# ZephirFXEC/HNanoSolver

Measured on AMD Instinct MI355X. Metric: solver substeps/sec (advect + 50 red-black SOR iterations + project) at N active voxels, higher is better.
Workload: dtype f32

## Files before the change

### hnanosolver_amd/csrc/hns_advect.hip

```cpp
#include <cstdlib>
#include <cstring>

#include "hns_device.hpp"

namespace hns {

struct Taps {
	int t[8];
	float fx, fy, fz;
};

constexpr unsigned kOutside = 0xFFFFE000u;
constexpr uint64_t kNarrowBytes = 0xFFFF0000ull;

__device__ __forceinline__ f3 ldv(const v4i& r, unsigned o4) {
	const v3f v = hns_buffer_load_v3f32(r, (int)(o4 + (o4 << 1)), 0, 0);
	return f3{v.x, v.y, v.z};
}
__device__ __forceinline__ float lds1(const v4i& r, unsigned o4) { return hns_buffer_load_f32(r, (int)o4, 0, 0); }

__device__ __forceinline__ void ld_zpair(const v4i& r, unsigned lo, unsigned hi, float& a, float& b) {
	const v2f32 v = hns_buffer_load_v2f32(r, (int)lo, 0, 0);
	a = v.x;
	b = v.y;
	if (hi != lo + 4u) b = lds1(r, hi);
}

struct GenericTabs {
	int nbr[27], base[27];
	__device__ __forceinline__ void set(int t, int nb) { nbr[t] = nb, base[t] = nb < 0 ? -1 : nb * 512; }
};
constexpr int kPadTab = 48;
struct NarrowTabs {
	int nbr[27];
	unsigned b4[27], b4p[kPadTab];
	__device__ __forceinline__ void set(int t, int nb) {
		const int ax = t / 9, ay = (t - 9 * ax) / 3, az = t - 9 * ax - 3 * ay;
		nbr[t] = nb, b4[t] = b4p[(ax * 4 + ay) * 4 + az] = nb < 0 ? kOutside : (unsigned)nb * 2048u;
	}
};

__device__ __forceinline__ int3 voxel_ijk(const int4 org, int n) { return int3{org.x + (n >> 6), org.y + ((n >> 3) & 7), org.z + (n & 7)}; }

template <class Tabs>
struct LeafVoxel {
	Tabs& tabs;
	const int n, leaf, idx;
	int4 org;
	int3 c;
	float px, py, pz;
	__device__ __forceinline__ LeafVoxel(const GridDev& g, Tabs& t) : tabs(t), n(threadIdx.x), leaf(launch_leaf(g, blockIdx.x)), idx(leaf * 512 + n) {}
	__device__ __forceinline__ void stage(const GridDev& g) {
		org = g.origins[leaf];
		if (threadIdx.x < 27) tabs.set(threadIdx.x, g.nbr27[leaf * 27 + threadIdx.x]);
		__syncthreads();
		c = voxel_ijk(org, n);
		px = (float)c.x, py = (float)c.y, pz = (float)c.z;
	}
};
typedef LeafVoxel<GenericTabs> GenericCtx;
typedef LeafVoxel<NarrowTabs> NarrowCtx;

__device__ __forceinline__ constexpr int tap_of(int q) { return ((q & 1) << 2) | (q & 2) | (q >> 2); }
template <int XS = 100, int YS = 10>
__device__ __forceinline__ constexpr int box_corner(int q) { return (q & 1) * XS + ((q >> 1) & 1) * YS + (q >> 2); }
__device__ __forceinline__ void tri_weights(float tx, float ty, float tz, float (&w)[8]) {
	const float itx = 1.0f - tx, ity = 1.0f - ty, itz = 1.0f - tz;
	const float w00 = itx * ity, w10 = tx * ity, w01 = itx * ty, w11 = tx * ty;
	w[0] = w00 * itz, w[1] = w10 * itz, w[2] = w01 * itz, w[3] = w11 * itz, w[4] = w00 * tz, w[5] = w10 * tz, w[6] = w01 * tz, w[7] = w11 * tz;
}
template <class T, class Lerp>
__device__ __forceinline__ T tri_nest_yx(const T (&z)[4], float fx, float fy, Lerp lerp) {
	const T y0 = lerp(z[0], z[1], fy), y1 = lerp(z[2], z[3], fy);
	return lerp(y0, y1, fx);
}
template <class T, class Lerp>
__device__ __forceinline__ T tri_nest(const T (&c)[8], float fx, float fy, float fz, Lerp lerp) {
	const T z[4] = {lerp(c[0], c[1], fz), lerp(c[2], c[3], fz), lerp(c[4], c[5], fz), lerp(c[6], c[7], fz)};
	return tri_nest_yx(z, fx, fy, lerp);
}
template <class T>
__device__ __forceinline__ T bfecc_limit(T phiOrig, const T (&nbr)[6], T phiForward, T phiCorr) {
	T mn = phiOrig, mx = phiOrig;
#pragma unroll
	for (int d = 0; d < 6; ++d) {
		mn = __builtin_elementwise_min(mn, nbr[d]);
		mx = __builtin_elementwise_max(mx, nbr[d]);
	}
	mn = __builtin_elementwise_min(mn, phiForward);
	mx = __builtin_elementwise_max(mx, phiForward);
	return __builtin_elementwise_max(mn, __builtin_elementwise_min(phiCorr, mx));
}
template <class Fetch>
__device__ __forceinline__ f3 bfecc_limit_v(const f3& vo, const f3& vf, const f3& vb, Fetch nbr) {
	float nx[6], ny[6], nz[6];
#pragma unroll
	for (int d = 0; d < 6; ++d) {
		const f3 t = nbr(d);
		nx[d] = t.x, ny[d] = t.y, nz[d] = t.z;
	}
	return f3{bfecc_limit(vo.x, nx, vf.x, vf.x + 0.5f * (vo.x - vb.x)), bfecc_limit(vo.y, ny, vf.y, vf.y + 0.5f * (vo.y - vb.y)),
	          bfecc_limit(vo.z, nz, vf.z, vf.z + 0.5f * (vo.z - vb.z))};
}

struct TapsB {
	unsigned o[8];
	float fx, fy, fz;
};

__device__ __forceinline__ Taps make_taps(const GridDev& g, const GenericCtx& C, float x, float y, float z) {
	Taps T;
	const int4 org = C.org;
	const int i = __float2int_rd(x), j = __float2int_rd(y), k = __float2int_rd(z);
	T.fx = x - (float)i;
	T.fy = y - (float)j;
	T.fz = z - (float)k;
	const int ax0 = (i >> 3) - (org.x >> 3) + 1, ax1 = ((i + 1) >> 3) - (org.x >> 3) + 1;
	const int ay0 = (j >> 3) - (org.y >> 3) + 1, ay1 = ((j + 1) >> 3) - (org.y >> 3) + 1;
	const int az0 = (k >> 3) - (org.z >> 3) + 1, az1 = ((k + 1) >> 3) - (org.z >> 3) + 1;
	const bool near = ((unsigned)ax0 <= 2u) & ((unsigned)ax1 <= 2u) & ((unsigned)ay0 <= 2u) & ((unsigned)ay1 <= 2u) & ((unsigned)az0 <= 2u) &
	                  ((unsigned)az1 <= 2u);
	if (near) {
		const int sx[2] = {ax0 * 9, ax1 * 9}, sy[2] = {ay0 * 3, ay1 * 3}, sz[2] = {az0, az1};
		const int lx[2] = {(i & 7) << 6, ((i + 1) & 7) << 6}, ly[2] = {(j & 7) << 3, ((j + 1) & 7) << 3}, lz[2] = {k & 7, (k + 1) & 7};
#pragma unroll
		for (int c = 0; c < 8; ++c) {
			const int di = c >> 2, dj = (c >> 1) & 1, dk = c & 1;
			const int b = C.tabs.base[sx[di] + sy[dj] + sz[dk]];
			T.t[c] = b < 0 ? -1 : b + (lx[di] | ly[dj] | lz[dk]);
		}
	} else {
		int any = 0;
		far_cell_taps(g, C.tabs.nbr, org, i, j, k, T.t);
#pragma unroll
		for (int c = 0; c < 8; ++c) any |= T.t[c];
		if (any < 0 && g.far_flag) *g.far_flag = 1;
	}
	return T;
}

__device__ __forceinline__ TapsB make_taps_b(const GridDev& g, const NarrowCtx& C, float x, float y, float z) {
	TapsB T;
	const int4 org = C.org;
	const int i = __float2int_rd(x), j = __float2int_rd(y), k = __float2int_rd(z);
	T.fx = x - (float)i;
	T.fy = y - (float)j;
	T.fz = z - (float)k;
	const unsigned dx = (unsigned)(i - (org.x - 8)), dy = (unsigned)(j - (org.y - 8)), dz = (unsigned)(k - (org.z - 8));
	if (max(dx, max(dy, dz)) < 23u) {
		const unsigned ex = dx + 1u, ey = dy + 1u, ez = dz + 1u;
		const unsigned X[2] = {(dx & 24u) << 3, (ex & 24u) << 3}, Y[2] = {(dy & 24u) << 1, (ey & 24u) << 1}, Z[2] = {(dz & 24u) >> 1, (ez & 24u) >> 1};
		const unsigned lx[2] = {(dx & 7u) << 8, (ex & 7u) << 8}, ly[2] = {(dy & 7u) << 5, (ey & 7u) << 5}, lz[2] = {(dz & 7u) << 2, (ez & 7u) << 2};
		const unsigned XY[4] = {X[0] | Y[0], X[0] | Y[1], X[1] | Y[0], X[1] | Y[1]};
		const unsigned lxy[4] = {lx[0] | ly[0], lx[0] | ly[1], lx[1] | ly[0], lx[1] | ly[1]};
// ... 174 lines not shown
	const v4i ru = field_rsrc(u, (unsigned)g.n_leaves * 6144u);
	const f3 vo = ldv(ru, (unsigned)C.idx << 2);
	C.stage(g);
	int cell;
	const unsigned off = box_shell_off<kVX, kVY>(tabs.b4, C.n, cell);
	velocity_box_store<kVP>(s_box, C.n, cell, velocity_box_load<kVX, kVY, kVP>(s_box, ru, C.n, vo, off));
	float sx = C.px - scaled_dt * vo.x, sy = C.py - scaled_dt * vo.y, sz = C.pz - scaled_dt * vo.z;
	f3 vf = {0.0f, 0.0f, 0.0f}, vb = {0.0f, 0.0f, 0.0f};
	__syncthreads();
#pragma unroll 1
	for (int pass = 0; pass < 2; ++pass) {
		const f3 v = sample_velocity(g, C, ru, s_box, sx, sy, sz);
		if (pass == 0) {
			vf = v;
			sx = sx + scaled_dt * v.x, sy = sy + scaled_dt * v.y, sz = sz + scaled_dt * v.z;
		} else {
			vb = v;
		}
	}
	const int ob = box_own<kVX, kVY>(C.n);
	st3(out, C.idx, bfecc_limit_v(vo, vf, vb, [&](int d) { return box_f3(s_box, ob + box_nbr<kVX, kVY>(d)); }));
}

template <bool COLL>
__global__ __launch_bounds__(512) void k_advect_vector(const GridDev g, const float* __restrict__ u, float* __restrict__ out,
                                                       const float* __restrict__ sdf, const float scaled_dt, const float inv_dx) {
	__shared__ GenericTabs tabs;
	GenericCtx C(g, tabs);
	C.stage(g);
	const int idx = C.idx;

	const f3 vo = ld3(u, idx);
	float sx = C.px - scaled_dt * vo.x, sy = C.py - scaled_dt * vo.y, sz = C.pz - scaled_dt * vo.z;
	float rx = C.px, ry = C.py, rz = C.pz;
	f3 vf = {0.0f, 0.0f, 0.0f}, vb = {0.0f, 0.0f, 0.0f};
#pragma unroll 1
	for (int pass = 0; pass < 2; ++pass) {
		Taps T = make_taps(g, C, sx, sy, sz);
		if (COLL) {
			if (tri_f_t(sdf, T) < 0.0f) {
				sx = rx, sy = ry, sz = rz;
				T = make_taps(g, C, sx, sy, sz);
			}
		}
		const f3 v = tri_v_t(u, T);
		if (pass == 0) {
			vf = v;
			rx = sx, ry = sy, rz = sz;
			sx = sx + scaled_dt * v.x, sy = sy + scaled_dt * v.y, sz = sz + scaled_dt * v.z;
		} else {
			vb = v;
		}
	}
	int nb[6];
	nbr6(tabs.base, C.leaf, C.n, nb);
	f3 vc = bfecc_limit_v(vo, vf, vb, [&](int d) { return ld3z(u, nb[d]); });

	if (COLL) {
		const float sv = sdf[idx];
		if (sv < 0.0f) {
			vc.x = vc.y = vc.z = 0.0f;
		} else if (sv < 0.1f) {
			const f3 nrm = sdf_normal(g, tabs.nbr, C.org, sdf, C.c.x, C.c.y, C.c.z, inv_dx);
			vc = no_slip_blend(vc, nrm, 1.0f - (sv / 1.5f));
		}
	}
	st3(out, idx, vc);
}


__global__ __launch_bounds__(512) void k_advect_scalar_n(const GridDev g, const float* __restrict__ u, const float* __restrict__ in, float* __restrict__ out,
                                                         const float scaled_dt) {
	__shared__ NarrowTabs tabs;
	NarrowCtx C(g, tabs);
	C.stage(g);
	const int n = C.n;
	const unsigned bytes1 = (unsigned)g.n_leaves * 2048u, own = (unsigned)C.idx << 2;
	const v4i ru = field_rsrc(u, bytes1 * 3u), rf = field_rsrc(in, bytes1);

	__shared__ float s_tile[kTile];
	const float phiOrig = lds1(rf, own);
	s_tile[n] = phiOrig;
	if (n < 384) s_tile[512 + n] = lds1(rf, halo_off(tabs.b4, n));
	const f3 vc = ldv(ru, own);
	float sx = C.px - scaled_dt * vc.x, sy = C.py - scaled_dt * vc.y, sz = C.pz - scaled_dt * vc.z;
	float phiForward = 0.0f, phiBackward = 0.0f;
#pragma unroll 1
	for (int pass = 0; pass < 2; ++pass) {
		const TapsB T = make_taps_b(g, C, sx, sy, sz);
		const float phi = tri_f_b(rf, T);
		if (pass == 0) {
			phiForward = phi;
			const f3 vf = tri_v_b(ru, T);
			sx = sx + scaled_dt * vf.x, sy = sy + scaled_dt * vf.y, sz = sz + scaled_dt * vf.z;
		} else {
			phiBackward = phi;
		}
	}
	const float error = phiOrig - phiBackward;
	__syncthreads();
	const float nv[6] = {s_tile[tile_nbr<0, -1>(n)], s_tile[tile_nbr<0, 1>(n)], s_tile[tile_nbr<1, -1>(n)], s_tile[tile_nbr<1, 1>(n)], s_tile[tile_nbr<2, -1>(n)], s_tile[tile_nbr<2, 1>(n)]};
	out[C.idx] = bfecc_limit(phiOrig, nv, phiForward, phiForward + 0.5f * error);
}

template <bool COLL>
__global__ __launch_bounds__(512) void k_advect_scalar(const GridDev g, const float* __restrict__ u, const float* __restrict__ in,
                                                       float* __restrict__ out, const float* __restrict__ sdf, const float scaled_dt) {
	__shared__ GenericTabs tabs;
	GenericCtx C(g, tabs);
	C.stage(g);
	const int idx = C.idx;

	const float phiOrig = in[idx];
	const f3 vc = ld3(u, idx);
	float sx = C.px - scaled_dt * vc.x, sy = C.py - scaled_dt * vc.y, sz = C.pz - scaled_dt * vc.z;
	float rx = C.px, ry = C.py, rz = C.pz;
	float phiForward = 0.0f, phiBackward = 0.0f;
#pragma unroll 1
	for (int pass = 0; pass < 2; ++pass) {
		Taps T = make_taps(g, C, sx, sy, sz);
		if (COLL) {
			if (tri_f_t(sdf, T) < 0.0f) {
				sx = rx, sy = ry, sz = rz;
				T = make_taps(g, C, sx, sy, sz);
			}
		}
		const float phi = tri_f_t(in, T);
		if (pass == 0) {
			phiForward = phi;
			const f3 vf = tri_v_t(u, T);
			rx = sx, ry = sy, rz = sz;
			sx = sx + scaled_dt * vf.x, sy = sy + scaled_dt * vf.y, sz = sz + scaled_dt * vf.z;
		} else {
			phiBackward = phi;
		}
	}
	const float error = phiOrig - phiBackward;
	int nb[6];
	nbr6(tabs.base, C.leaf, C.n, nb);
	float nv[6];
#pragma unroll
	for (int d = 0; d < 6; ++d) nv[d] = ldz(in, nb[d]);
	out[idx] = bfecc_limit(phiOrig, nv, phiForward, phiForward + 0.5f * error);
}


#define HNS_MAX_SCALARS 8
struct ScalarPtrs {
	const float* in[HNS_MAX_SCALARS];
	float* out[HNS_MAX_SCALARS];
	int n;
	const float* q4;
	float* q4_out[4];
};

__device__ __forceinline__ void interp_from_taps(const Taps& T, int oob, int (&ix)[8], float (&w)[8]) {
	tri_weights(T.fx, T.fy, T.fz, w);
#pragma unroll
	for (int q = 0; q < 8; ++q) ix[q] = T.t[tap_of(q)] < 0 ? oob : T.t[tap_of(q)];
}
__device__ __forceinline__ void add_weighted(f3& a, const f3& v, float w) { a.x = a.x + w * v.x, a.y = a.y + w * v.y, a.z = a.z + w * v.z; }

template <bool BOX>
__device__ __forceinline__ bool sample_setup(const GridDev& g, const NarrowCtx& C, float x, float y, float z, unsigned oob4, int& cell, unsigned (&o)[8], float (&w)[8]) {
	const int i = __float2int_rd(x), j = __float2int_rd(y), k = __float2int_rd(z);
	const unsigned rx = (unsigned)(i - (C.org.x - 1)), ry = (unsigned)(j - (C.org.y - 1)), rz = (unsigned)(k - (C.org.z - 1));
	const bool boxed = BOX && max(rx, max(ry, rz)) <= 8u;
	cell = boxed ? (int)((rx * 10u + ry) * 10u + rz) : 0;
	float tx, ty, tz;
	if (boxed) {
		tx = x - (float)i, ty = y - (float)j, tz = z - (float)k;
#pragma unroll
		for (int q = 0; q < 8; ++q) o[q] = 0u;
	} else {
		const TapsB T = make_taps_b(g, C, x, y, z);
		tx = T.fx, ty = T.fy, tz = T.fz;
#pragma unroll
		for (int q = 0; q < 8; ++q) o[q] = T.o[tap_of(q)] >= kOutside ? oob4 : T.o[tap_of(q)];
	}
	tri_weights(tx, ty, tz, w);
	return boxed;
}

template <bool Q4, bool AHEAD = false>
__global__ __launch_bounds__(512) __attribute__((amdgpu_waves_per_eu(Q4 || AHEAD ? 6 : 4))) void k_advect_scalars_n(const GridDev g, const float* __restrict__ u, const ScalarPtrs P, const float scaled_dt,
                                                                                                            float* __restrict__ adv_out) {
	static_assert(!(Q4 && AHEAD), "the look-ahead form is float-only");
	__shared__ NarrowTabs tabs;
	NarrowCtx C(g, tabs);
	const int n = C.n, idx = C.idx;
	const unsigned bytes1 = (unsigned)g.n_leaves * 2048u;
	const v4i ru = field_rsrc(u, bytes1 * 3u);
	const unsigned own = (unsigned)idx << 2, oob4 = (unsigned)g.oob << 2;
	const f3 vc = ldv(ru, own);
	C.stage(g);

	const int ob = box_own(n);
	int hcell;
	unsigned ho = box_shell_off(tabs.b4, n, hcell);
	ho = ho >= kOutside ? oob4 : ho;
	constexpr bool FIRST = Q4;
	__shared__ float s_ubox[FIRST ? 3 * kBox : 1];
	if constexpr (FIRST) velocity_box_store<kBox>(s_ubox, n, hcell, velocity_box_load<100, 10, kBox>(s_ubox, ru, n, vc, ho));

	const float bx = C.px - scaled_dt * vc.x, by = C.py - scaled_dt * vc.y, bz = C.pz - scaled_dt * vc.z;
	unsigned bo[8], fo[8];
	float bw[8], fw[8];
	bool bboxed = false;
	int ba = 0;
	f3 vf = {0.0f, 0.0f, 0.0f};
	__shared__ float s_vbox[AHEAD ? 3 * kVP : 1];
	__shared__ float s_wf[AHEAD ? 3 * 512 : 1];
	if constexpr (AHEAD) {
		int vcell;
		const unsigned voff = box_shell_off<kVX, kVY>(tabs.b4, n, vcell);
		const f3 hv = velocity_box_load<kVX, kVY, kVP>(s_vbox, ru, n, vc, voff);
		const TapsB T = make_taps_b(g, C, bx, by, bz);
		V3 c[8];
#pragma unroll
		for (int q = 0; q < 8; ++q) {
			const v3f v = hns_buffer_load_v3f32(ru, (int)(T.o[tap_of(q)] + (T.o[tap_of(q)] << 1)), 0, 0);
			c[tap_of(q)].xy = v2f32{v.x, v.y};
			c[tap_of(q)].z = v.z;
		}
		const float* __restrict__ uoob = u + 3 * (size_t)g.oob;
		const f3 uo = {uoob[0], uoob[1], uoob[2]};
		velocity_box_store<kVP>(s_vbox, n, vcell, hv);
		tri_weights(T.fx, T.fy, T.fz, bw);
		V3 z[4];
#pragma unroll
		for (int q = 0; q < 8; ++q) {
			const int t = tap_of(q);
			const bool outside = T.o[t] >= kOutside;
			bo[q] = outside ? oob4 : T.o[t];
			add_weighted(vf, f3{outside ? uo.x : c[t].xy.x, outside ? uo.y : c[t].xy.y, outside ? uo.z : c[t].z}, bw[q]);
			if (t & 1) z[t >> 1] = lerp_v3(c[t - 1], c[t], T.fz);
		}
		const V3 r = tri_nest_yx(z, T.fx, T.fy, lerp_v3);
		s_wf[n] = r.xy.x, s_wf[n + 512] = r.xy.y, s_wf[n + 1024] = r.z;
	} else {
		bboxed = sample_setup<FIRST>(g, C, bx, by, bz, oob4, ba, bo, bw);
		f3 vt[8];
		if (!bboxed) {
#pragma unroll
			for (int q = 0; q < 8; ++q) vt[q] = ldv(ru, bo[q]);
		}
		if constexpr (FIRST) __syncthreads();
		if (bboxed) {
#pragma unroll
			for (int q = 0; q < 8; ++q) {
				const int a = ba + box_corner(q);
				vt[q] = f3{s_ubox[a], s_ubox[a + kBox], s_ubox[a + 2 * kBox]};
			}
		}
#pragma unroll
		for (int q = 0; q < 8; ++q) add_weighted(vf, vt[q], bw[q]);
	}
	int fa;
	const bool boxed = sample_setup<true>(g, C, bx + scaled_dt * vf.x, by + scaled_dt * vf.y, bz + scaled_dt * vf.z, oob4, fa, fo, fw);
	__shared__ float s_box[2][kBox];
	if constexpr (Q4) {
		__shared__ v4f32 s_box4[kBox];
		const v4i rq = field_rsrc(P.q4, bytes1 * 4u);
		const v4f32 phiOrig = hns_buffer_load_v4f32(rq, (int)(own << 2), 0, 0);
		s_box4[ob] = phiOrig;
		if (n < kBoxShell) s_box4[hcell] = hns_buffer_load_v4f32(rq, (int)(ho << 2), 0, 0);
		v4f32 phiF = {0.0f, 0.0f, 0.0f, 0.0f}, phiB = {0.0f, 0.0f, 0.0f, 0.0f};
		if (!bboxed) {
			v4f32 c[8];
#pragma unroll
			for (int q = 0; q < 8; ++q) c[q] = hns_buffer_load_v4f32(rq, (int)(bo[q] << 2), 0, 0);
#pragma unroll
			for (int q = 0; q < 8; ++q) phiF = __builtin_elementwise_fma(c[q], v4f32{bw[q], bw[q], bw[q], bw[q]}, phiF);
		}
		if (!boxed) {
			v4f32 c[8];
#pragma unroll
			for (int q = 0; q < 8; ++q) c[q] = hns_buffer_load_v4f32(rq, (int)(fo[q] << 2), 0, 0);
#pragma unroll
			for (int q = 0; q < 8; ++q) phiB = __builtin_elementwise_fma(c[q], v4f32{fw[q], fw[q], fw[q], fw[q]}, phiB);
		}
		__syncthreads();
		if (bboxed) {
#pragma unroll
			for (int q = 0; q < 8; ++q) phiF = __builtin_elementwise_fma(s_box4[ba + box_corner(q)], v4f32{bw[q], bw[q], bw[q], bw[q]}, phiF);
		}
		if (boxed) {
#pragma unroll
			for (int q = 0; q < 8; ++q) phiB = __builtin_elementwise_fma(s_box4[fa + box_corner(q)], v4f32{fw[q], fw[q], fw[q], fw[q]}, phiB);
		}
		v4f32 nv[6];
#pragma unroll
		for (int d = 0; d < 6; ++d) nv[d] = s_box4[ob + box_nbr(d)];
		const v4f32 r = bfecc_limit(phiOrig, nv, phiF, __builtin_elementwise_fma(v4f32{0.5f, 0.5f, 0.5f, 0.5f}, phiOrig - phiB, phiF));
		P.q4_out[0][idx] = r.x, P.q4_out[1][idx] = r.y, P.q4_out[2][idx] = r.z, P.q4_out[3][idx] = r.w;
	}
	for (int s = 0; s < P.n; ++s) {
		const v4i rf = field_rsrc(P.in[s], bytes1);
		float* box = s_box[s & 1];
		const float phiOrig = lds1(rf, own);
		box[ob] = phiOrig;
		if (n < kBoxShell) box[hcell] = lds1(rf, ho);
		float vb[8], vf8[8];
		if (!bboxed) {
#pragma unroll
			for (int q = 0; q < 4; ++q) ld_zpair(rf, bo[q], bo[q + 4], vb[q], vb[q + 4]);
		}
		if (!boxed) {
#pragma unroll
			for (int q = 0; q < 4; ++q) ld_zpair(rf, fo[q], fo[q + 4], vf8[q], vf8[q + 4]);
		}
		float phiF = 0.0f, phiB = 0.0f;
		__syncthreads();
		if (bboxed) {
#pragma unroll
			for (int q = 0; q < 8; ++q) vb[q] = box[ba + box_corner(q)];
		}
#pragma unroll
		for (int q = 0; q < 8; ++q) phiF = __fmaf_rn(vb[q], bw[q], phiF);
		if (boxed) {
#pragma unroll
			for (int q = 0; q < 8; ++q) vf8[q] = box[fa + box_corner(q)];
		}
#pragma unroll
		for (int q = 0; q < 8; ++q) phiB = __fmaf_rn(vf8[q], fw[q], phiB);
		float nv[6];
#pragma unroll
		for (int d = 0; d < 6; ++d) nv[d] = box[ob + box_nbr(d)];
		P.out[s][idx] = bfecc_limit(phiOrig, nv, phiF, __fmaf_rn(0.5f, phiOrig - phiB, phiF));
	}
	if constexpr (AHEAD) {
		__syncthreads();
		int m = n;
		asm volatile("" : "+v"(m));
		const int obv = box_own<kVX, kVY>(m);
		const int3 w = voxel_ijk(C.org, m);
		const f3 vo = box_f3(s_vbox, obv);
		const f3 wf = f3{s_wf[m], s_wf[m + 512], s_wf[m + 1024]};
		const float cx = (float)w.x - scaled_dt * vo.x, cy = (float)w.y - scaled_dt * vo.y, cz = (float)w.z - scaled_dt * vo.z;
		const f3 wb = sample_velocity(g, C, ru, s_vbox, cx + scaled_dt * wf.x, cy + scaled_dt * wf.y, cz + scaled_dt * wf.z);
		st3(adv_out, idx, bfecc_limit_v(vo, wf, wb, [&](int d) { return box_f3(s_vbox, obv + box_nbr<kVX, kVY>(d)); }));
	}
}

template <bool COLL>
__global__ __launch_bounds__(512) void k_advect_scalars(const GridDev g, const float* __restrict__ u, const ScalarPtrs P,
                                                        const float* __restrict__ sdf, const float scaled_dt) {
	__shared__ GenericTabs tabs;
	GenericCtx C(g, tabs);
	C.stage(g);
	const int idx = C.idx;

	const f3 vc = ld3(u, idx);
	float sx = C.px - scaled_dt * vc.x, sy = C.py - scaled_dt * vc.y, sz = C.pz - scaled_dt * vc.z;
	float rx = C.px, ry = C.py, rz = C.pz;
	int bi[8], fi[8];
	float bw[8], fw[8];
#pragma unroll 1
	for (int pass = 0; pass < 2; ++pass) {
		Taps T = make_taps(g, C, sx, sy, sz);
		if (COLL) {
			if (tri_f_t(sdf, T) < 0.0f) {
				sx = rx, sy = ry, sz = rz;
				T = make_taps(g, C, sx, sy, sz);
			}
		}
		if (pass == 0) {
			interp_from_taps(T, g.oob, bi, bw);
			f3 vf = {0.0f, 0.0f, 0.0f};
#pragma unroll
			for (int q = 0; q < 8; ++q) add_weighted(vf, ld3(u, bi[q]), bw[q]);
			rx = sx, ry = sy, rz = sz;
			sx = sx + scaled_dt * vf.x, sy = sy + scaled_dt * vf.y, sz = sz + scaled_dt * vf.z;
		} else {
			interp_from_taps(T, g.oob, fi, fw);
		}
	}
	int nb[6];
	nbr6(tabs.base, C.leaf, C.n, nb);
#pragma unroll
	for (int d = 0; d < 6; ++d) nb[d] = nb[d] < 0 ? g.oob : nb[d];
	for (int s = 0; s < P.n; ++s) {
		const float* __restrict__ in = P.in[s];
		const float phiOrig = in[idx];
		float phiF = 0.0f, phiB = 0.0f;
#pragma unroll
		for (int q = 0; q < 8; ++q) {
			phiF = __fmaf_rn(in[bi[q]], bw[q], phiF);
			phiB = __fmaf_rn(in[fi[q]], fw[q], phiB);
		}
		float nv[6];
#pragma unroll
		for (int d = 0; d < 6; ++d) nv[d] = in[nb[d]];
		P.out[s][idx] = bfecc_limit(phiOrig, nv, phiF, __fmaf_rn(0.5f, phiOrig - phiB, phiF));
	}
}

}

using namespace hns;

static bool narrow_fields(const hns_grid* g) {
	return !options().advect_generic.load() && (uint64_t)g->topo.n_leaves * 6144u <= hns::kNarrowBytes;
}

enum class AdvectForm { collision, narrow, generic };
static AdvectForm advect_form(const hns_grid* g, const float* sdf, int has_collision) {
	return has_collision && sdf ? AdvectForm::collision : (narrow_fields(g) ? AdvectForm::narrow : AdvectForm::generic);
}

static GridDev reversed(const hns_grid* g) {
	GridDev gd = g->dev();
	gd.rev = 1;
	return gd;
}

static int fill_scalar_ptrs(ScalarPtrs& P, const float* const* in, float* const* out, int n) {
	int bad = -1;
	P.n = n;
	P.q4 = nullptr, P.q4_out[0] = P.q4_out[1] = P.q4_out[2] = P.q4_out[3] = nullptr;
	for (int s = 0; s < HNS_MAX_SCALARS; ++s) {
		P.in[s] = s < n ? in[s] : nullptr;
		P.out[s] = s < n ? out[s] : nullptr;
		if (s < n && (!P.in[s] || !P.out[s]) && bad < 0) bad = s;
	}
	return bad;
}

extern "C" {

int hns_dev_advect_vector(hns_grid* g, const float* vel3, float* out3, const float* sdf, int has_collision, float dt, float inv_dx, void* stream) {
	if (int rc = check_grid(g, "hns_dev_advect_vector")) return rc;
	NULLCHK(!vel3 || !out3, "hns_dev_advect_vector");
	if (vel3 == out3) return fail(HNS_ERR_INVALID_ARGUMENT, "hns_dev_advect_vector: output must not alias input");
	if (g->n_active == 0) return HNS_OK;
	const float scaled_dt = dt * inv_dx;
	const dim3 grid((unsigned)g->n_active), block(512);
	switch (advect_form(g, sdf, has_collision)) {
	case AdvectForm::collision: hipLaunchKernelGGL(k_advect_vector<true>, grid, block, 0, (hipStream_t)stream, g->dev(), vel3, out3, sdf, scaled_dt, inv_dx); break;
	case AdvectForm::narrow: hipLaunchKernelGGL(k_advect_vector_n, grid, block, 0, (hipStream_t)stream, g->dev(), vel3, out3, scaled_dt); break;
	case AdvectForm::generic: hipLaunchKernelGGL(k_advect_vector<false>, grid, block, 0, (hipStream_t)stream, g->dev(), vel3, out3, sdf, scaled_dt, inv_dx); break;
	}
	return launch_status("hns_dev_advect_vector");
}

int hns_dev_advect_scalar(hns_grid* g, const float* vel3, const float* in, float* out, const float* sdf, int has_collision, float dt, float inv_dx,
                          void* stream) {
	if (int rc = check_grid(g, "hns_dev_advect_scalar")) return rc;
	NULLCHK(!vel3 || !in || !out, "hns_dev_advect_scalar");
	if (g->n_active == 0) return HNS_OK;
	const float scaled_dt = dt * inv_dx;
	const dim3 grid((unsigned)g->n_active), block(512);
	switch (advect_form(g, sdf, has_collision)) {
	case AdvectForm::collision: hipLaunchKernelGGL(k_advect_scalar<true>, grid, block, 0, (hipStream_t)stream, g->dev(), vel3, in, out, sdf, scaled_dt); break;
	case AdvectForm::narrow: hipLaunchKernelGGL(k_advect_scalar_n, grid, block, 0, (hipStream_t)stream, g->dev(), vel3, in, out, scaled_dt); break;
	case AdvectForm::generic: hipLaunchKernelGGL(k_advect_scalar<false>, grid, block, 0, (hipStream_t)stream, g->dev(), vel3, in, out, sdf, scaled_dt); break;
	}
	return launch_status("hns_dev_advect_scalar");
}

int hns_dev_advect_scalars(hns_grid* g, const float* vel3, const float* const* in, float* const* out, int n, const float* sdf, int has_collision,
                           float dt, float inv_dx, void* stream) {
	if (int rc = check_grid(g, "hns_dev_advect_scalars")) return rc;
	NULLCHK(!vel3 || (n > 0 && (!in || !out)), "hns_dev_advect_scalars");
	if (g->n_active == 0 || n <= 0) return HNS_OK;
	const float scaled_dt = dt * inv_dx;
	const dim3 grid((unsigned)g->n_active), block(512);
	for (int base = 0; base < n; base += HNS_MAX_SCALARS) {
		ScalarPtrs P;
		const int bad = fill_scalar_ptrs(P, in + base, out + base, n - base < HNS_MAX_SCALARS ? n - base : HNS_MAX_SCALARS);
		if (bad >= 0) {
			set_error("hns_dev_advect_scalars: null device pointer for field %d", base + bad);
			return HNS_ERR_INVALID_ARGUMENT;
		}
		switch (advect_form(g, sdf, has_collision)) {
		case AdvectForm::collision: hipLaunchKernelGGL(k_advect_scalars<true>, grid, block, 0, (hipStream_t)stream, g->dev(), vel3, P, sdf, scaled_dt); break;
		case AdvectForm::narrow: hipLaunchKernelGGL(k_advect_scalars_n<false>, grid, block, 0, (hipStream_t)stream, reversed(g), vel3, P, scaled_dt, (float*)nullptr); break;
		case AdvectForm::generic: hipLaunchKernelGGL(k_advect_scalars<false>, grid, block, 0, (hipStream_t)stream, g->dev(), vel3, P, sdf, scaled_dt); break;
		}
	}
	return launch_status("hns_dev_advect_scalars");
}

bool hns_advect_ahead_ok(const hns_grid* g) { return narrow_fields(g); }

int hns_dev_advect_scalars_ahead(hns_grid* g, const float* vel3, const float* const* in, float* const* out, int n, float* adv_out3, float dt, float inv_dx, void* stream) {
	if (int rc = check_grid(g, "hns_dev_advect_scalars_ahead")) return rc;
	NULLCHK(!vel3 || !adv_out3 || (n > 0 && (!in || !out)), "hns_dev_advect_scalars_ahead");
	if (vel3 == adv_out3) return fail(HNS_ERR_INVALID_ARGUMENT, "hns_dev_advect_scalars_ahead: adv_out3 must not alias vel3");
	if (n < 0 || n > HNS_MAX_SCALARS) return fail(HNS_ERR_INVALID_ARGUMENT, "hns_dev_advect_scalars_ahead: between 0 and 8 fields");
	if (!narrow_fields(g)) return fail(HNS_ERR_INVALID_ARGUMENT, "hns_dev_advect_scalars_ahead: grid too large for 32-bit offsets (or option advect = generic)");
	if (g->n_active == 0) return HNS_OK;
	ScalarPtrs P;
	const int bad = fill_scalar_ptrs(P, in, out, n);
	if (bad >= 0) {
		set_error("hns_dev_advect_scalars_ahead: null device pointer for field %d", bad);
		return HNS_ERR_INVALID_ARGUMENT;
	}
	hipLaunchKernelGGL((k_advect_scalars_n<false, true>), dim3((unsigned)g->n_active), dim3(512), 0, (hipStream_t)stream, reversed(g), vel3, P, dt * inv_dx, adv_out3);
	return launch_status("hns_dev_advect_scalars_ahead");
}

int hns_advect_scalars_q4(hns_grid* g, const float* vel3, const float* q4, float* const* q4_out, const float* const* in, float* const* out, int n, float dt, float inv_dx,
                          void* stream) {
	if (int rc = check_grid(g, "hns_advect_scalars_q4")) return rc;
	NULLCHK(!vel3 || !q4 || !q4_out || (n > 0 && (!in || !out)), "hns_advect_scalars_q4");
	if (!hns_advect_q4_ok(g) || n > HNS_MAX_SCALARS) return fail(HNS_ERR_INVALID_ARGUMENT, "hns_advect_scalars_q4: grid too large for 32-bit offsets, or too many fields");
	if (g->n_active == 0) return HNS_OK;
	for (int c = 0; c < 4; ++c) NULLCHK(!q4_out[c], "hns_advect_scalars_q4");
	ScalarPtrs P;
	NULLCHK(fill_scalar_ptrs(P, in, out, n) >= 0, "hns_advect_scalars_q4");
	P.q4 = q4;
	for (int c = 0; c < 4; ++c) P.q4_out[c] = q4_out[c];
	hipLaunchKernelGGL(k_advect_scalars_n<true>, dim3((unsigned)g->n_active), dim3(512), 0, (hipStream_t)stream, reversed(g), vel3, P, dt * inv_dx, (float*)nullptr);
	return launch_status("hns_advect_scalars_q4");
}

bool hns_advect_q4_ok(const hns_grid* g) { return narrow_fields(g) && (uint64_t)g->topo.n_leaves * 8192u <= hns::kNarrowBytes; }

}
```

### hnanosolver_amd/csrc/hns_internal.hpp

```cpp
#pragma once

#include <hip/hip_runtime.h>

#include <algorithm>
#include <atomic>
#include <cstdarg>
#include <cstdint>
#include <cstdio>
#include <mutex>
#include <string>
#include <vector>

#include "hns.h"

namespace hns {

void set_error(const char* fmt, ...);
inline int fail(int code, const char* msg) {
	set_error("%s", msg);
	return code;
}

#define HNS_TRY(call)                    \
	do {                                 \
		int rc__ = (call);               \
		if (rc__ != HNS_OK) return rc__; \
	} while (0)

#define HNS_HIP(call)                                                                                   \
	do {                                                                                                \
		hipError_t e__ = (call);                                                                        \
		if (e__ != hipSuccess) {                                                                        \
			hns::set_error("%s failed: %s (%s:%d)", #call, hipGetErrorString(e__), __FILE__, __LINE__); \
			return HNS_ERR_HIP;                                                                         \
		}                                                                                               \
	} while (0)

constexpr const char* kCombustionFields[4] = {"fuel", "waste", "temperature", "flame"};

struct EventGroups {
	size_t per;
	std::vector<hipEvent_t> ev;
	size_t used = 0;
	bool on = false;
	explicit EventGroups(size_t per_) : per(per_) {}
	int reset(int groups) {
		while (ev.size() < (size_t)groups * per) {
			hipEvent_t e;
			HNS_HIP(hipEventCreate(&e));
			ev.push_back(e);
		}
		on = groups > 0;
		used = 0;
		return HNS_OK;
	}
	hipEvent_t* current() { return on && (used + 1) * per <= ev.size() ? &ev[used * per] : nullptr; }
	void advance() { ++used; }
	int elapsed(double* ms) {
		std::fill(ms, ms + per - 1, 0.0);
		for (size_t g = 0; g < used; ++g) {
			const hipEvent_t* e = &ev[g * per];
			HNS_HIP(hipEventSynchronize(e[per - 1]));
			for (size_t k = 0; k + 1 < per; ++k) {
				float t = 0.0f;
				HNS_HIP(hipEventElapsedTime(&t, e[k], e[k + 1]));
				ms[k] += t;
			}
		}
		return HNS_OK;
	}
	void destroy() {
		for (hipEvent_t e : ev) (void)hipEventDestroy(e);
		ev.clear();
	}
};

struct DeviceScope {
	int prev = -1;
	bool switched = false;
	explicit DeviceScope(int device) {
		if (device >= 0 && hipGetDevice(&prev) == hipSuccess && prev != device) switched = hipSetDevice(device) == hipSuccess;
	}
	~DeviceScope() {
		if (switched) (void)hipSetDevice(prev);
	}
};

enum { kRbgsAuto = 0, kRbgsColor = 1 };
enum { kScheduleAuto = 0, kScheduleLinear = 1 };
enum { kLookaheadAuto = 0, kLookaheadOff = 1, kLookaheadOn = 2 };
struct Options {
	std::atomic<int> rbgs{kRbgsAuto};
	std::atomic<int> advect_generic{0};
	std::atomic<int> stencil_block{0};
	std::atomic<int> schedule{kScheduleAuto};
	std::atomic<int> cook_cache{1};
	std::atomic<int> cook_pipeline{1};
	std::atomic<int> divergence_form{0};
	std::atomic<int> fuse_pointwise{1};
	std::atomic<int> lookahead{kLookaheadAuto};
	std::atomic<int> sor_block_lb{0};
	std::atomic<int> dist_wire_us{0};
	std::atomic<int> dist_mirror{1};
	std::atomic<int> arena_fill{-1};
	std::atomic<int> dist_unsplit{1};
};
Options& options();

struct Topology {
	std::vector<int32_t> origins;
	std::vector<int32_t> nbr27;
	std::vector<int32_t> hash;
	uint32_t hash_mask = 0;
	int64_t n_leaves = 0;
	bool have_tables = false;

	int prepare(const int32_t* leaf_origins_xyz, int64_t n_leaves);
	int build_tables();
	int64_t find_leaf(int32_t ox, int32_t oy, int32_t oz) const;
	uint64_t offset(int32_t i, int32_t j, int32_t k) const;
};

uint32_t hash_origin(int32_t x, int32_t y, int32_t z);
void sort_leaf_origins(int32_t* xyz, size_t n);

struct GridDev {
	const int4* origins;
	const int* nbr27;
	const int* hash;
	const int* sched;
	int sched_seg;
	int sched_pre;
	const int* blk;
	uint32_t hash_mask;
	int n_leaves;
	int n_active;
	int first;
	int oob;
	int rev;
	int* far_flag;
};

__device__ __forceinline__ unsigned launch_pos(const GridDev& g, unsigned b) {
	if (!g.rev) return b;
	const unsigned rows = (unsigned)g.n_active >> 3;
	return (b >> 3) < rows ? (((rows - 1u - (b >> 3)) << 3) | (b & 7u)) : b;
}

__device__ __forceinline__ int launch_leaf(const GridDev& g, unsigned b) {
	const int pos = (int)launch_pos(g, b);
	if (g.sched_seg == 0 && g.sched_pre == 0) {
		const int base = g.n_active >> 3, rem = g.n_active & 7, x = pos & 7, i = pos >> 3;
		return g.first + x * base + (x < rem ? x : rem) + i;
	}
	return g.sched ? g.sched[pos] : g.first + pos;
}

}

struct hns_sim;

struct hns_grid {
	hns::Topology topo;
	float voxel_size = 1.0f;
	uint64_t n_active = 0;
	uint64_t first_active = 0;
	uint64_t outside_element = 0;
	int* far_flag = nullptr;
	bool on_device = false;
	int device = -1;
	void* d_origins = nullptr;
	void* d_nbr27 = nullptr;
	void* d_hash = nullptr;
	void* d_sched = nullptr;
	void* d_blk = nullptr;
	int sched_seg = -1, sched_pre = 0;
	uint64_t chain_boundary = 0;
	uint64_t sched_prefix = 0;
	void* d_sched_mem = nullptr;
	void* d_scratch = nullptr;
	void* d_arena = nullptr;
	size_t arena_bytes = 0;
	void* d_sb_tab = nullptr;
	size_t sb_bytes = 0;
	uint64_t n_sb = 0;
	bool sb_built = false;
	int sb_seg = 0;
	uint64_t sb_first = 0, sb_count = 0;
	std::vector<std::pair<void*, size_t>> sb_retired;
	void* d_diag = nullptr;
	size_t diag_bytes = 0;
	std::mutex build_mutex;
	std::mutex host_mutex;
	std::vector<hns_sim*> sim_cache;
	hns::GridDev dev() const;
};

struct hns_sim {
	hns_grid* grid = nullptr;
	uint64_t n = 0;
	std::vector<std::string> names;
	std::vector<float*> cur;
	std::vector<float*> nxt;
	float* vel = nullptr;
	float* adv = nullptr;
	float* tmp = nullptr;
	float* q4 = nullptr;
	float* div = nullptr;
	float* p_a = nullptr;
	float* p_b = nullptr;
	float* p_result = nullptr;
	hns::EventGroups solve_ev{2};
	long long timed_launches = 0;
	hns::EventGroups stage_ev{6};
	hipStream_t xfer = nullptr;
	hipEvent_t xev[5] = {nullptr, nullptr, nullptr, nullptr, nullptr};
	bool cached = false, in_use = false;
	struct Handed { uint64_t sig = 0, dig = 0; };
	Handed handed_vel;
	std::vector<Handed> handed_cur;
	static constexpr int kVelocity = -1, kEverything = -2;
	struct Ahead {
		bool valid = false;
		const hns_grid* grid = nullptr;
		uint64_t first = 0, n_active = 0;
		uint32_t dt_bits = 0, vs_bits = 0;
	};
	Ahead ahead;
	bool ahead_off = false;
	bool have_last = false;
	uint32_t last_dt_bits = 0, last_vs_bits = 0;
	long long ahead_produced = 0, ahead_consumed = 0;
	void drop_ahead() { ahead.valid = false; }
	void forget(int k = kEverything) {
		drop_ahead();
		if (k == kEverything || k == kVelocity) handed_vel = Handed{};
		for (size_t i = 0; i < handed_cur.size(); ++i)
			if (k == kEverything || k == (int)i) handed_cur[i] = Handed{};
	}
	unsigned long long* d_dig = nullptr;
	unsigned long long* h_dig = nullptr;
	void* arena = nullptr;
	size_t arena_bytes = 0;
	unsigned char* d_masks = nullptr;
	size_t masks_bytes = 0;
	hipEvent_t rev[6] = {nullptr, nullptr, nullptr, nullptr, nullptr, nullptr};
	bool regrid_timed = false;
	void* d_act = nullptr;
	size_t act_bytes = 0;
	void* d_diag = nullptr;
	size_t diag_bytes = 0;
	hns_stats* h_diag = nullptr;
	bool solved = false;
// ... 64 lines not shown
```

### hnanosolver_amd/csrc/hns_topology.cpp

```cpp
#include <cstdlib>
#include <cstring>
#include <thread>

#include "hns_internal.hpp"

namespace hns {

static thread_local std::string g_last_error;

void set_error(const char* fmt, ...) {
	char buf[1024];
	va_list ap;
	va_start(ap, fmt);
	vsnprintf(buf, sizeof(buf), fmt, ap);
	va_end(ap);
	g_last_error = buf;
}

Options& options() {
	static Options o;
	return o;
}

uint32_t hash_origin(int32_t x, int32_t y, int32_t z) {
	uint32_t h = (uint32_t)(x >> 3) * 0x9E3779B1u;
	h ^= (uint32_t)(y >> 3) * 0x85EBCA77u;
	h ^= (uint32_t)(z >> 3) * 0xC2B2AE3Du;
	h ^= h >> 15;
	h *= 0x2C1B3C6Du;
	h ^= h >> 12;
	return h;
}

int64_t Topology::find_leaf(int32_t ox, int32_t oy, int32_t oz) const {
	if (n_leaves == 0) return -1;
	uint32_t s = hash_origin(ox, oy, oz) & hash_mask;
	for (;;) {
		const int32_t l = hash[s];
		if (l < 0) return -1;
		const int32_t* o = &origins[4 * (size_t)l];
		if (o[0] == ox && o[1] == oy && o[2] == oz) return l;
		s = (s + 1) & hash_mask;
	}
}

uint64_t Topology::offset(int32_t i, int32_t j, int32_t k) const {
	const int64_t l = find_leaf(i & ~7, j & ~7, k & ~7);
	if (l < 0) return 0;
	return (uint64_t)l * 512u + (uint64_t)(((i & 7) << 6) | ((j & 7) << 3) | (k & 7)) + 1u;
}

int Topology::prepare(const int32_t* leaf_origins_xyz, int64_t n) {
	if (n < 0 || n > (int64_t(1) << 22)) {
		set_error("hns_grid: %lld leaves exceeds the 2^22-leaf (2^31-voxel) limit of 32-bit voxel indices", (long long)n);
		return HNS_ERR_TOPOLOGY;
	}
	n_leaves = n;
	have_tables = false;
	origins.assign((size_t)n * 4, 0);
	uint32_t size = 16;
	while ((int64_t)size < 2 * n + 2) size <<= 1;
	hash_mask = size - 1;
	for (int64_t l = 0; l < n; ++l) {
		const int32_t ox = leaf_origins_xyz[3 * l], oy = leaf_origins_xyz[3 * l + 1], oz = leaf_origins_xyz[3 * l + 2];
		if ((ox & 7) || (oy & 7) || (oz & 7)) {
			set_error("hns_grid: leaf %lld origin (%d,%d,%d) is not 8-aligned: coordinates are not leaf-dense", (long long)l, ox, oy, oz);
			return HNS_ERR_TOPOLOGY;
		}
		origins[4 * l] = ox;
		origins[4 * l + 1] = oy;
		origins[4 * l + 2] = oz;
	}
	return HNS_OK;
}

int Topology::build_tables() {
	const int64_t n = n_leaves;
	hash.assign((size_t)hash_mask + 1, -1);
	for (int64_t l = 0; l < n; ++l) {
		const int32_t ox = origins[4 * l], oy = origins[4 * l + 1], oz = origins[4 * l + 2];
		uint32_t s = hash_origin(ox, oy, oz) & hash_mask;
		while (hash[s] >= 0) {
			const int32_t* o = &origins[4 * (size_t)hash[s]];
			if (o[0] == ox && o[1] == oy && o[2] == oz) {
				set_error("hns_grid: leaf origin (%d,%d,%d) appears twice (leaves %d and %lld)", ox, oy, oz, hash[s], (long long)l);
				return HNS_ERR_TOPOLOGY;
			}
			s = (s + 1) & hash_mask;
		}
		hash[s] = (int32_t)l;
	}
	nbr27.assign((size_t)n * 27, -1);
	for (int64_t l = 0; l < n; ++l) {
		const int32_t* o = &origins[4 * (size_t)l];
		for (int dx = -1; dx <= 1; ++dx)
			for (int dy = -1; dy <= 1; ++dy)
				for (int dz = -1; dz <= 1; ++dz) {
					const int64_t nx = (int64_t)o[0] + 8 * dx, ny = (int64_t)o[1] + 8 * dy, nz = (int64_t)o[2] + 8 * dz;
					int64_t nb = -1;
					if (nx >= INT32_MIN && nx <= INT32_MAX && ny >= INT32_MIN && ny <= INT32_MAX && nz >= INT32_MIN && nz <= INT32_MAX)
						nb = find_leaf((int32_t)nx, (int32_t)ny, (int32_t)nz);
					nbr27[(size_t)l * 27 + (dx + 1) * 9 + (dy + 1) * 3 + (dz + 1)] = (int32_t)nb;
				}
	}
	have_tables = true;
	return HNS_OK;
}

}

using namespace hns;

extern "C" {

const char* hns_last_error(void) { return g_last_error.c_str(); }
int hns_version(void) { return HNS_VERSION; }

namespace {
struct OptionDesc {
	const char* name;
	std::atomic<int> Options::*field;
	const char* const* words;
	int max = 1 << 20;
	const char* off = nullptr;
};
const char* const kWordsRbgs[] = {"auto", "color", nullptr};
const char* const kWordsAdvect[] = {"auto", "generic", nullptr};
const char* const kWordsStencil[] = {"auto", "block", nullptr};
const char* const kWordsSchedule[] = {"auto", "linear", nullptr};
const char* const kWordsBool[] = {"0", "1", nullptr};
const char* const kWordsMirror[] = {"0", "1", "guarded", nullptr};
const char* const kWordsUnsplit[] = {"0", "1", "always", nullptr};
const char* const kWordsDivergence[] = {"auto", "row", "coalesced", "zpair", nullptr};
const char* const kWordsLookahead[] = {"auto", "0", "1", nullptr};
const OptionDesc kOptions[] = {
    {"rbgs", &Options::rbgs, kWordsRbgs},
    {"advect", &Options::advect_generic, kWordsAdvect},
    {"stencil", &Options::stencil_block, kWordsStencil},
    {"schedule", &Options::schedule, kWordsSchedule},
    {"cook_cache", &Options::cook_cache, kWordsBool},
    {"cook_pipeline", &Options::cook_pipeline, kWordsBool},
    {"divergence", &Options::divergence_form, kWordsDivergence},
    {"fuse", &Options::fuse_pointwise, kWordsBool},
    {"lookahead", &Options::lookahead, kWordsLookahead},
    {"sor_block_lb", &Options::sor_block_lb, nullptr},
    {"dist_wire_us", &Options::dist_wire_us, nullptr},
    {"dist_mirror", &Options::dist_mirror, kWordsMirror},
    {"dist_unsplit", &Options::dist_unsplit, kWordsUnsplit},
    {"arena_fill", &Options::arena_fill, nullptr, 255, "off"},
};
const Options kDefaults;
}

int hns_set_option(const char* name, const char* value) {
	if (!name) return fail(HNS_ERR_INVALID_ARGUMENT, "hns_set_option: null name");
	for (const OptionDesc& d : kOptions) {
		if (strcmp(d.name, name) != 0) continue;
		if (!value) {
			(options().*d.field).store((kDefaults.*d.field).load());
			return HNS_OK;
		}
		if (!d.words) {
			if (d.off && strcmp(d.off, value) == 0) {
				(options().*d.field).store(-1);
				return HNS_OK;
			}
			char* end = nullptr;
			const long v = strtol(value, &end, 10);
			if (end == value || *end || v < 0 || v > d.max) break;
			(options().*d.field).store((int)v);
			return HNS_OK;
		}
		for (int i = 0; d.words[i]; ++i)
			if (strcmp(d.words[i], value) == 0) {
				(options().*d.field).store(i);
				return HNS_OK;
			}
		break;
	}
	set_error("hns_set_option: unknown option or value: %s = %s", name, value ? value : "(default)");
	return HNS_ERR_INVALID_ARGUMENT;
}

const char* hns_get_option(const char* name) {
	static thread_local char buf[16];
	if (!name) return nullptr;
	for (const OptionDesc& d : kOptions) {
		if (strcmp(d.name, name) != 0) continue;
		const int v = (options().*d.field).load();
		if (d.words) return d.words[v];
		if (d.off && v < 0) return d.off;
		snprintf(buf, sizeof(buf), "%d", v);
		return buf;
	}
	return nullptr;
}

static hns_grid* grid_from_origins(const int32_t* origins, uint64_t n_leaves, float voxel_size, unsigned flags, int* err) {
	int rc = HNS_OK;
	hns_grid* g = new hns_grid;
	g->voxel_size = voxel_size;
	rc = g->topo.prepare(origins, (int64_t)n_leaves);
	if (rc == HNS_OK) {
		g->n_active = n_leaves;
		rc = (flags & HNS_GRID_HOST_ONLY) ? g->topo.build_tables() : hns_grid_upload(g);
	}
	if (rc != HNS_OK) {
		hns_grid_free_device(g);
		delete g;
		g = nullptr;
	}
	if (err) *err = rc;
	return g;
}

hns_grid* hns_grid_create_from_leaves(const int32_t* leaf_origins_xyz, uint64_t n_leaves, float voxel_size, unsigned flags, int* err) {
	if (!leaf_origins_xyz && n_leaves) {
		if (err) *err = fail(HNS_ERR_INVALID_ARGUMENT, "hns_grid_create_from_leaves: null origin array");
		return nullptr;
	}
	return grid_from_origins(leaf_origins_xyz, n_leaves, voxel_size, flags, err);
}

static int scan_coords(const char* who, const int32_t* coords, uint64_t n_voxels, unsigned flags, std::vector<int32_t>& origins) {
	if (!coords && n_voxels) {
		set_error("%s: null coordinate array", who);
		return HNS_ERR_INVALID_ARGUMENT;
	}
	if (n_voxels % 512u) {
		set_error("%s: %llu coordinates is not a multiple of 512: the domain must be leaf-dense", who, (unsigned long long)n_voxels);
		return HNS_ERR_TOPOLOGY;
	}
	const uint64_t n_leaves = n_voxels / 512u;
	origins.resize((size_t)n_leaves * 3);
	const bool validate = !(flags & HNS_GRID_SKIP_VALIDATE);
	unsigned n_threads = 1;
	if (validate && n_leaves >= 2048) {
		n_threads = std::thread::hardware_concurrency();
		if (n_threads == 0) n_threads = 1;
		if (n_threads > 16) n_threads = 16;
	}
	std::vector<uint64_t> first_bad(n_threads, UINT64_MAX);
	auto scan = [&](unsigned t) {
		const uint64_t l0 = n_leaves * t / n_threads, l1 = n_leaves * (t + 1) / n_threads;
		for (uint64_t l = l0; l < l1; ++l) {
			const int32_t* c = coords + 3 * 512 * l;
			origins[3 * l] = c[0];
			origins[3 * l + 1] = c[1];
			origins[3 * l + 2] = c[2];
			if (!validate || first_bad[t] != UINT64_MAX) continue;
			for (int n = 1; n < 512; ++n) {
				const int32_t* v = c + 3 * n;
				if (v[0] != c[0] + (n >> 6) || v[1] != c[1] + ((n >> 3) & 7) || v[2] != c[2] + (n & 7)) {
					first_bad[t] = 512 * l + n;
					break;
				}
			}
		}
	};
	if (n_threads == 1) {
		scan(0);
	} else {
		std::vector<std::thread> pool;
		for (unsigned t = 1; t < n_threads; ++t) pool.emplace_back(scan, t);
		scan(0);
		for (auto& th : pool) th.join();
	}
	for (unsigned t = 0; t < n_threads; ++t) {
		if (first_bad[t] == UINT64_MAX) continue;
		const uint64_t i = first_bad[t];
		const int32_t* v = coords + 3 * i;
		set_error("%s: coordinate %llu = (%d,%d,%d) breaks the leaf-dense x<<6|y<<3|z order of leaf %llu", who, (unsigned long long)i, v[0], v[1], v[2],
		          (unsigned long long)(i / 512));
		return HNS_ERR_TOPOLOGY;
	}
	return HNS_OK;
}

hns_grid* hns_grid_create(const int32_t* coords, uint64_t n_voxels, float voxel_size, unsigned flags, int* err) {
	std::vector<int32_t> origins;
	const int rc = scan_coords("hns_grid_create", coords, n_voxels, flags, origins);
	if (rc != HNS_OK) {
		if (err) *err = rc;
		return nullptr;
	}
	return grid_from_origins(origins.data(), n_voxels / 512u, voxel_size, flags, err);
}

int hns_grid_matches(const hns_grid* g, const int32_t* coords, uint64_t n_voxels, unsigned flags) {
	if (!g) return fail(HNS_ERR_INVALID_ARGUMENT, "hns_grid_matches: null grid");
	std::vector<int32_t> origins;
	const int rc = scan_coords("hns_grid_matches", coords, n_voxels, flags, origins);
	if (rc != HNS_OK) return rc;
	const uint64_t n_leaves = n_voxels / 512u;
	if (n_leaves != (uint64_t)g->topo.n_leaves) return 0;
	for (uint64_t l = 0; l < n_leaves; ++l) {
		const int32_t* o = &g->topo.origins[4 * (size_t)l];
// ... 69 lines not shown
```

Baseline: 646.5.

## Sample back-trace velocity from shared box in lookahead advect and stage first scalar

In the lookahead advection kernel, adds an opt-in path: when the whole wavefront's back-traced points fall inside the staged velocity box and all neighbor leaves exist, velocity is interpolated from shared memory instead of global buffer loads. Independently, the first scalar field's own and halo values are loaded early and stored to the shared box before a single shared barrier. This removes one barrier in the scalar loop and another before the epilogue. The box path is off by default via a new option, and the restructured barriers add correctness risk around shared-memory reuse.

```diff
diff --git a/hnanosolver_amd/csrc/hns_advect.hip b/hnanosolver_amd/csrc/hns_advect.hip
--- a/hnanosolver_amd/csrc/hns_advect.hip
+++ b/hnanosolver_amd/csrc/hns_advect.hip
@@ -1,5 +1,6 @@
 #include <cstdlib>
 #include <cstring>
+#include <type_traits>
 
 #include "hns_device.hpp"
 
@@ -480,6 +481,7 @@
 	int n;
 	const float* q4;
 	float* q4_out[4];
+	int back_box;
 };
 
 __device__ __forceinline__ void interp_from_taps(const Taps& T, int oob, int (&ix)[8], float (&w)[8]) {
@@ -539,33 +541,67 @@
 	f3 vf = {0.0f, 0.0f, 0.0f};
 	__shared__ float s_vbox[AHEAD ? 3 * kVP : 1];
 	__shared__ float s_wf[AHEAD ? 3 * 512 : 1];
+	__shared__ float s_box[2][kBox];
 	if constexpr (AHEAD) {
 		int vcell;
 		const unsigned voff = box_shell_off<kVX, kVY>(tabs.b4, n, vcell);
 		const f3 hv = velocity_box_load<kVX, kVY, kVP>(s_vbox, ru, n, vc, voff);
-		const TapsB T = make_taps_b(g, C, bx, by, bz);
+		float p0 = 0.0f, h0 = 0.0f;
+		if (P.n > 0) {
+			const v4i rf = field_rsrc(P.in[0], bytes1);
+			p0 = lds1(rf, own);
+			if (n < kBoxShell) h0 = lds1(rf, ho);
+		}
+		const unsigned lane = (unsigned)n & 63u;
+		const bool full = __all(tabs.b4[lane < 27u ? lane : 13u] < kOutside);
+		const int bi = __float2int_rd(bx), bj = __float2int_rd(by), bk = __float2int_rd(bz);
+		const unsigned rx = (unsigned)bi - (unsigned)(C.org.x - 1), ry = (unsigned)bj - (unsigned)(C.org.y - 1), rz = (unsigned)bk - (unsigned)(C.org.z - 1);
+		const bool fast = P.back_box && full && __all(max(rx, max(ry, rz)) <= 8u);
+		auto two_samples = [&](auto mapped, const V3(&c)[8], const unsigned(&o)[8], const f3& uo, float fx, float fy, float fz) {
+			tri_weights(fx, fy, fz, bw);
+			V3 z[4];
+#pragma unroll
+			for (int q = 0; q < 8; ++q) {
+				const int t = tap_of(q);
+				const bool outside = decltype(mapped)::value && o[t] >= kOutside;
+				bo[q] = outside ? oob4 : o[t];
+				add_weighted(vf, f3{outside ? uo.x : c[t].xy.x, outside ? uo.y : c[t].xy.y, outside ? uo.z : c[t].z}, bw[q]);
+				if (t & 1) z[t >> 1] = lerp_v3(c[t - 1], c[t], fz);
+			}
+			const V3 r = tri_nest_yx(z, fx, fy, lerp_v3);
+			s_wf[n] = r.xy.x, s_wf[n + 512] = r.xy.y, s_wf[n + 1024] = r.z;
+		};
+		TapsB T;
 		V3 c[8];
-#pragma unroll
-		for (int q = 0; q < 8; ++q) {
-			const v3f v = hns_buffer_load_v3f32(ru, (int)(T.o[tap_of(q)] + (T.o[tap_of(q)] << 1)), 0, 0);
-			c[tap_of(q)].xy = v2f32{v.x, v.y};
-			c[tap_of(q)].z = v.z;
-		}
-		const float* __restrict__ uoob = u + 3 * (size_t)g.oob;
-		const f3 uo = {uoob[0], uoob[1], uoob[2]};
+		f3 uo = {0.0f, 0.0f, 0.0f};
+		if (!fast) {
+			T = make_taps_b(g, C, bx, by, bz);
+#pragma unroll
+			for (int q = 0; q < 8; ++q) {
+				const v3f v = hns_buffer_load_v3f32(ru, (int)(T.o[tap_of(q)] + (T.o[tap_of(q)] << 1)), 0, 0);
+				c[tap_of(q)].xy = v2f32{v.x, v.y};
+				c[tap_of(q)].z = v.z;
+			}
+			const float* __restrict__ uoob = u + 3 * (size_t)g.oob;
+			uo = f3{uoob[0], uoob[1], uoob[2]};
+		}
 		velocity_box_store<kVP>(s_vbox, n, vcell, hv);
-		tri_weights(T.fx, T.fy, T.fz, bw);
-		V3 z[4];
-#pragma unroll
-		for (int q = 0; q < 8; ++q) {
-			const int t = tap_of(q);
-			const bool outside = T.o[t] >= kOutside;
-			bo[q] = outside ? oob4 : T.o[t];
-			add_weighted(vf, f3{outside ? uo.x : c[t].xy.x, outside ? uo.y : c[t].xy.y, outside ? uo.z : c[t].z}, bw[q]);
-			if (t & 1) z[t >> 1] = lerp_v3(c[t - 1], c[t], T.fz);
-		}
-		const V3 r = tri_nest_yx(z, T.fx, T.fy, lerp_v3);
-		s_wf[n] = r.xy.x, s_wf[n + 512] = r.xy.y, s_wf[n + 1024] = r.z;
+		if (P.n > 0) {
+			s_box[0][ob] = p0;
+			if (n < kBoxShell) s_box[0][hcell] = h0;
+		}
+		__syncthreads();
+		if (fast) {
+			V3 cb[8];
+			const unsigned none[8] = {0u, 0u, 0u, 0u, 0u, 0u, 0u, 0u};
+			const int va = (int)(rx * (unsigned)kVX + ry * (unsigned)kVY + rz);
+#pragma unroll
+			for (int q = 0; q < 8; ++q) cb[tap_of(q)] = box_v3(s_vbox, va + box_corner<kVX, kVY>(q));
+			two_samples(std::false_type{}, cb, none, uo, bx - (float)bi, by - (float)bj, bz - (float)bk);
+			bboxed = true, ba = (int)((rx * 10u + ry) * 10u + rz);
+		} else {
+			two_samples(std::true_type{}, c, T.o, uo, T.fx, T.fy, T.fz);
+		}
 	} else {
 		bboxed = sample_setup<FIRST>(g, C, bx, by, bz, oob4, ba, bo, bw);
 		f3 vt[8];
@@ -586,7 +622,6 @@
 	}
 	int fa;
 	const bool boxed = sample_setup<true>(g, C, bx + scaled_dt * vf.x, by + scaled_dt * vf.y, bz + scaled_dt * vf.z, oob4, fa, fo, fw);
-	__shared__ float s_box[2][kBox];
 	if constexpr (Q4) {
 		__shared__ v4f32 s_box4[kBox];
 		const v4i rq = field_rsrc(P.q4, bytes1 * 4u);
@@ -626,9 +661,13 @@
 	for (int s = 0; s < P.n; ++s) {
 		const v4i rf = field_rsrc(P.in[s], bytes1);
 		float* box = s_box[s & 1];
-		const float phiOrig = lds1(rf, own);
-		box[ob] = phiOrig;
-		if (n < kBoxShell) box[hcell] = lds1(rf, ho);
+		const bool staged = AHEAD && s == 0;
+		float phiOrig = 0.0f;
+		if (!staged) {
+			phiOrig = lds1(rf, own);
+			box[ob] = phiOrig;
+			if (n < kBoxShell) box[hcell] = lds1(rf, ho);
+		}
 		float vb[8], vf8[8];
 		if (!bboxed) {
 #pragma unroll
@@ -639,7 +678,8 @@
 			for (int q = 0; q < 4; ++q) ld_zpair(rf, fo[q], fo[q + 4], vf8[q], vf8[q + 4]);
 		}
 		float phiF = 0.0f, phiB = 0.0f;
-		__syncthreads();
+		if (!staged) __syncthreads();
+		if (staged) phiOrig = box[ob];
 		if (bboxed) {
 #pragma unroll
 			for (int q = 0; q < 8; ++q) vb[q] = box[ba + box_corner(q)];
@@ -658,7 +698,6 @@
 		P.out[s][idx] = bfecc_limit(phiOrig, nv, phiF, __fmaf_rn(0.5f, phiOrig - phiB, phiF));
 	}
 	if constexpr (AHEAD) {
-		__syncthreads();
 		int m = n;
 		asm volatile("" : "+v"(m));
 		const int obv = box_own<kVX, kVY>(m);
@@ -747,6 +786,7 @@
 	int bad = -1;
 	P.n = n;
 	P.q4 = nullptr, P.q4_out[0] = P.q4_out[1] = P.q4_out[2] = P.q4_out[3] = nullptr;
+	P.back_box = 0;
 	for (int s = 0; s < HNS_MAX_SCALARS; ++s) {
 		P.in[s] = s < n ? in[s] : nullptr;
 		P.out[s] = s < n ? out[s] : nullptr;
@@ -825,6 +865,7 @@
 		set_error("hns_dev_advect_scalars_ahead: null device pointer for field %d", bad);
 		return HNS_ERR_INVALID_ARGUMENT;
 	}
+	P.back_box = options().lookahead_box.load();
 	hipLaunchKernelGGL((k_advect_scalars_n<false, true>), dim3((unsigned)g->n_active), dim3(512), 0, (hipStream_t)stream, reversed(g), vel3, P, dt * inv_dx, adv_out3);
 	return launch_status("hns_dev_advect_scalars_ahead");
 }
diff --git a/hnanosolver_amd/csrc/hns_internal.hpp b/hnanosolver_amd/csrc/hns_internal.hpp
--- a/hnanosolver_amd/csrc/hns_internal.hpp
+++ b/hnanosolver_amd/csrc/hns_internal.hpp
@@ -99,6 +99,7 @@
 	std::atomic<int> divergence_form{0};
 	std::atomic<int> fuse_pointwise{1};
 	std::atomic<int> lookahead{kLookaheadAuto};
+	std::atomic<int> lookahead_box{0};
 	std::atomic<int> sor_block_lb{0};
 	std::atomic<int> dist_wire_us{0};
 	std::atomic<int> dist_mirror{1};
diff --git a/hnanosolver_amd/csrc/hns_topology.cpp b/hnanosolver_amd/csrc/hns_topology.cpp
--- a/hnanosolver_amd/csrc/hns_topology.cpp
+++ b/hnanosolver_amd/csrc/hns_topology.cpp
@@ -143,6 +143,7 @@
     {"divergence", &Options::divergence_form, kWordsDivergence},
     {"fuse", &Options::fuse_pointwise, kWordsBool},
     {"lookahead", &Options::lookahead, kWordsLookahead},
+    {"lookahead_box", &Options::lookahead_box, kWordsBool},
     {"sor_block_lb", &Options::sor_block_lb, nullptr},
     {"dist_wire_us", &Options::dist_wire_us, nullptr},
     {"dist_mirror", &Options::dist_mirror, kWordsMirror},
```

New measurement: 646.9 (median of 5 runs). About the same (+0.1%).
